# nmichlo/mtg-vision

Hardware: AMD Instinct MI355X
Metric: cards/sec end-to-end (detect+embed+top-1 over 100k bank), 640x640 (higher is better)
Workload: dtype f32 (products as 3 x f16 MFMA on hi/lo-split operands, f32 accumulate)

## Files before the change

mtg-vision_amd/csrc/dwconv7_ln_kernel.h:

```cpp
#pragma once
#include "common.h"
#include "dwconv7_ln_stream_kernel.h"
#include "sp8.h"

namespace mtgv {

typedef float f32x4 __attribute__((ext_vector_type(4)));

template <int TW, bool SP8, int PK, bool WL = false>
__global__ __launch_bounds__(256) void dwconv7_ln_kernel(const float* __restrict__ in, const float* __restrict__ w49,
                                                        const float* __restrict__ bias, const float* __restrict__ ln_w,
                                                        const float* __restrict__ ln_b, float* __restrict__ out, int H, int W,
                                                        int C, int nstrips, long total_strips, int S, float eps) {
  extern __shared__ __attribute__((aligned(16))) float sm[];
  const int c4n = C >> 2;
  float* part = sm;
  float* stat = sm + S * TW * c4n;
  const float* wl = w49;
  long blk;
  {
    const long nwg = gridDim.x, b = blockIdx.x;
    const long q = nwg >> 3, r = nwg & 7, x = b & 7;
    blk = (x < r ? x * (q + 1) : r * (q + 1) + (x - r) * q) + (b >> 3);
  }
  const int tid = threadIdx.x;
  if (WL) {
    float* wdst = stat + ((S * TW * 2 + 3) & ~3);
    for (int i = tid; i < 49 * c4n; i += 256) reinterpret_cast<f32x4*>(wdst)[i] = reinterpret_cast<const f32x4*>(w49)[i];
    wl = wdst;
    __syncthreads();
  }
  const int sl = tid / c4n, c4 = tid % c4n;
  const long strip = blk * S + sl;
  const bool live = sl < S && strip < total_strips;
  const int c = c4 * 4;
  int ws = 0, h = 0;
  long n = 0;
  if (live) {
    ws = (int)(strip % nstrips);
    const long t = strip / nstrips;
    h = (int)(t % H);
    n = t / H;
  }
  const int w0 = ws * TW;
  f32x4 acc[TW];
  if (live) {
    const f32x4 bv = *reinterpret_cast<const f32x4*>(bias + c);
#pragma unroll
    for (int j = 0; j < TW; ++j) acc[j] = bv;
#ifndef DW_DBG
#define DW_DBG 0
#endif
#pragma unroll 1
    for (int kh = 0; kh < 7; ++kh) {
      const int ih = h + kh - 3;
      if (ih < 0 || ih >= H) continue;
      if (DW_DBG == 1 && kh != 3) continue;
      const float* rowp = in + ((n * H + ih) * W) * C + c;
      f32x4 r[TW + 6];
#pragma unroll
      for (int j = 0; j < TW + 6; ++j) {
        const int iw = w0 + j - 3;
        f32x4 v = {0.f, 0.f, 0.f, 0.f};
        if (iw >= 0 && iw < W) v = *reinterpret_cast<const f32x4*>(rowp + (long)iw * C);
        r[j] = v;
      }
#pragma unroll
      for (int kw = 0; kw < 7; ++kw) {
        const f32x4 wv = *reinterpret_cast<const f32x4*>(wl + (kh * 7 + kw) * C + c);
#pragma unroll
        for (int j = 0; j < TW; ++j) {
          if (DW_DBG == 2) acc[j] += (kw == 0 ? r[j] + r[j + 6] : wv);
          else acc[j] += r[j + kw] * wv;
        }
      }
    }
#pragma unroll
    for (int j = 0; j < TW; ++j) part[(sl * c4n + c4) * TW + j] = (acc[j][0] + acc[j][1]) + (acc[j][2] + acc[j][3]);
  }
  __syncthreads();
  if (live && c4 < TW) {
    const float* pp = part + sl * c4n * TW + c4;
    float sum = 0.f;
    for (int i = 0; i < c4n; ++i) sum += pp[i * TW];
    stat[(sl * TW + c4) * 2] = sum / (float)C;
  }
  __syncthreads();
  if (live) {
#pragma unroll
    for (int j = 0; j < TW; ++j) {
      const f32x4 d = acc[j] - stat[(sl * TW + j) * 2];
      part[(sl * c4n + c4) * TW + j] = (d[0] * d[0] + d[1] * d[1]) + (d[2] * d[2] + d[3] * d[3]);
    }
  }
  __syncthreads();
  if (live && c4 < TW) {
    const float* pp = part + sl * c4n * TW + c4;
    float sq = 0.f;
    for (int i = 0; i < c4n; ++i) sq += pp[i * TW];
    stat[(sl * TW + c4) * 2 + 1] = 1.0f / sqrtf(sq / (float)C + eps);
  }
  __syncthreads();
  if (live) {
    const f32x4 wv = *reinterpret_cast<const f32x4*>(ln_w + c);
    const f32x4 bv = *reinterpret_cast<const f32x4*>(ln_b + c);
    float* op = out + ((n * H + h) * W + w0) * C + c;
#pragma unroll
    for (int j = 0; j < TW; ++j)
      if (w0 + j < W) {
        const float mean = stat[(sl * TW + j) * 2], rstd = stat[(sl * TW + j) * 2 + 1];
        const f32x4 o = (acc[j] - mean) * rstd * wv + bv;
        if (SP8)
          *reinterpret_cast<sp_h8*>(reinterpret_cast<char*>(op + (long)j * C - c) + (c4 >> 1) * 32 + (c4 & 1) * 16) =
              sp8_piece_from_quad(o, c4);
        else
          *reinterpret_cast<f32x4*>(op + (long)j * C) = o;
      }
  }
}


template <int TW, int TH, bool SP8, bool WL = false>
__global__ __launch_bounds__(256) void dwconv7_ln_rows_kernel(const float* __restrict__ in, const float* __restrict__ w49,
                                                             const float* __restrict__ bias, const float* __restrict__ ln_w,
                                                             const float* __restrict__ ln_b, float* __restrict__ out, int H, int W,
                                                             int C, int nstrips, int nhg, long total_strips, int S, float eps) {
  extern __shared__ __attribute__((aligned(16))) float sm[];
  constexpr int P = TH * TW;
  const int c4n = C >> 2;
  float* part = sm;
  float* stat = sm + S * P * c4n;
  const float* wl = w49;
  const int tid = threadIdx.x;
  if (WL) {
    float* wdst = stat + ((S * P * 2 + 3) & ~3);
    for (int i = tid; i < 49 * c4n; i += 256) reinterpret_cast<f32x4*>(wdst)[i] = reinterpret_cast<const f32x4*>(w49)[i];
    wl = wdst;
    __syncthreads();
  }
  const int sl = tid / c4n, c4 = tid % c4n;
  const int c = c4 * 4;
  long blk;
  {
    const long nwg = gridDim.x, b = blockIdx.x;
    const long q = nwg >> 3, r = nwg & 7, x = b & 7;
    blk = (x < r ? x * (q + 1) : r * (q + 1) + (x - r) * q) + (b >> 3);
  }
  const long strip = blk * S + sl;
  const bool live = sl < S && strip < total_strips;
  int ws = 0, h0 = 0;
  long n = 0;
  if (live) {
    ws = (int)(strip % nstrips);
    const long t = strip / nstrips;
    h0 = (int)(t % nhg) * TH;
    n = t / nhg;
  }
  const int w0 = ws * TW;
  f32x4 acc[TH][TW];
  if (live) {
    const f32x4 bv = *reinterpret_cast<const f32x4*>(bias + c);
#pragma unroll
    for (int t = 0; t < TH; ++t)
#pragma unroll
      for (int j = 0; j < TW; ++j) acc[t][j] = bv;
#pragma unroll 1
    for (int ir = 0; ir < TH + 6; ++ir) {
      const int ih = h0 + ir - 3;
      if (ih < 0 || ih >= H) continue;
      const float* rowp = in + ((n * H + ih) * W) * C + c;
      f32x4 r[TW + 6];
#pragma unroll
      for (int j = 0; j < TW + 6; ++j) {
        const int iw = w0 + j - 3;
        f32x4 v = {0.f, 0.f, 0.f, 0.f};
        if (iw >= 0 && iw < W) v = *reinterpret_cast<const f32x4*>(rowp + (long)iw * C);
        r[j] = v;
      }
#pragma unroll
      for (int t = 0; t < TH; ++t) {
        const int kh = ir - t;
        if (kh < 0 || kh > 6) continue;
#pragma unroll
        for (int kw = 0; kw < 7; ++kw) {
          const f32x4 wv = *reinterpret_cast<const f32x4*>(wl + (kh * 7 + kw) * C + c);
#pragma unroll
          for (int j = 0; j < TW; ++j) acc[t][j] += r[j + kw] * wv;
        }
      }
    }
#pragma unroll
    for (int t = 0; t < TH; ++t)
#pragma unroll
      for (int j = 0; j < TW; ++j)
        part[(sl * c4n + c4) * P + t * TW + j] = (acc[t][j][0] + acc[t][j][1]) + (acc[t][j][2] + acc[t][j][3]);
  }
  __syncthreads();
  if (live)
    for (int p = c4; p < P; p += c4n) {
      const float* pp = part + sl * c4n * P + p;
      float sum = 0.f;
      for (int i = 0; i < c4n; ++i) sum += pp[i * P];
      stat[(sl * P + p) * 2] = sum / (float)C;
    }
  __syncthreads();
  if (live) {
#pragma unroll
    for (int t = 0; t < TH; ++t)
#pragma unroll
      for (int j = 0; j < TW; ++j) {
        const f32x4 d = acc[t][j] - stat[(sl * P + t * TW + j) * 2];
        part[(sl * c4n + c4) * P + t * TW + j] = (d[0] * d[0] + d[1] * d[1]) + (d[2] * d[2] + d[3] * d[3]);
      }
  }
  __syncthreads();
  if (live)
    for (int p = c4; p < P; p += c4n) {
      const float* pp = part + sl * c4n * P + p;
      float sq = 0.f;
      for (int i = 0; i < c4n; ++i) sq += pp[i * P];
      stat[(sl * P + p) * 2 + 1] = 1.0f / sqrtf(sq / (float)C + eps);
    }
  __syncthreads();
  if (live) {
    const f32x4 wv = *reinterpret_cast<const f32x4*>(ln_w + c);
    const f32x4 bv = *reinterpret_cast<const f32x4*>(ln_b + c);
#pragma unroll
    for (int t = 0; t < TH; ++t) {
      if (h0 + t >= H) continue;
      float* op = out + ((n * H + h0 + t) * W + w0) * C + c;
#pragma unroll
      for (int j = 0; j < TW; ++j)
        if (w0 + j < W) {
          const float mean = stat[(sl * P + t * TW + j) * 2], rstd = stat[(sl * P + t * TW + j) * 2 + 1];
          const f32x4 o = (acc[t][j] - mean) * rstd * wv + bv;
          if (SP8)
            *reinterpret_cast<sp_h8*>(reinterpret_cast<char*>(op + (long)j * C - c) + (c4 >> 1) * 32 + (c4 & 1) * 16) =
                sp8_piece_from_quad(o, c4);
          else
            *reinterpret_cast<f32x4*>(op + (long)j * C) = o;
        }
    }
  }
}

template <int TW, int TH, bool SP8, bool WL = false>
static void dwconv7_ln_rows_launch(const float* in, const float* w49, const float* bias, const float* ln_w, const float* ln_b,
                                   float* out, int N, int H, int W, int C, float eps, hipStream_t s) {
  const int nstrips = ceil_div(W, TW), nhg = ceil_div(H, TH);
  const int c4n = C / 4;
  const int S = 256 / c4n;
  const long total_strips = (long)N * nhg * nstrips;
  const unsigned grid = (unsigned)((total_strips + S - 1) / S);
  const size_t lds = (size_t)(S * TH * TW * (c4n + 2) + 4 + (WL ? 49 * C : 0)) * sizeof(float);
  if (lds > 65536) {
    static bool attr[MTGV_MAX_DEVICES] = {};
    const int dev = current_device();
    if (!attr[dev]) {
      HIP_OK(hipFuncSetAttribute(reinterpret_cast<const void*>(&dwconv7_ln_rows_kernel<TW, TH, SP8, WL>), hipFuncAttributeMaxDynamicSharedMemorySize, 160 * 1024));
      attr[dev] = true;
    }
  }
  hipLaunchKernelGGL((dwconv7_ln_rows_kernel<TW, TH, SP8, WL>), dim3(grid), dim3(256), lds, s, in, w49, bias, ln_w, ln_b, out, H, W, C,
                     nstrips, nhg, total_strips, S, eps);
  HIP_OK(hipGetLastError());
}

template <int PK>
static void dwconv7_ln_launch_t(const float* in, const float* w49, const float* bias, const float* ln_w, const float* ln_b,
                                float* out, int N, int H, int W, int C, float eps, hipStream_t s, int out_fmt) {
  const char* const rows_env = getenv("MTGV_DW_ROWS");
  const bool rows_on = !(rows_env && atoi(rows_env) == 0);
  if constexpr (PK == 0)
  if (rows_on && N >= 128) {
#define DWSTREAM_GO(C_, G_)                                                                                                \
  (out_fmt == 1 ? dwconv7_ln_stream_launch<C_, G_, 4, 3, true>(in, w49, bias, ln_w, ln_b, out, N, H, 1, eps, s)            \
                : dwconv7_ln_stream_launch<C_, G_, 4, 3, false>(in, w49, bias, ln_w, ln_b, out, N, H, 1, eps, s))
    if (C == 96 && W == 32) { DWSTREAM_GO(96, 8); return; }
    if (C == 192 && W == 16) { DWSTREAM_GO(192, 4); return; }
#undef DWSTREAM_GO
  }
  if constexpr (PK == 0)
  if (rows_on && W >= 4) {
    const int c4n_ = C / 4, S_ = 256 / c4n_;
    const bool table = (size_t)(S_ * 12 * (c4n_ + 2) + 4 + 49 * C) * sizeof(float) <= 65536;
#define DWROWS_GO(TW_, WL_)                                                                                          \
  (out_fmt == 1 ? dwconv7_ln_rows_launch<TW_, 3, true, WL_>(in, w49, bias, ln_w, ln_b, out, N, H, W, C, eps, s)        \
                : dwconv7_ln_rows_launch<TW_, 3, false, WL_>(in, w49, bias, ln_w, ln_b, out, N, H, W, C, eps, s))
    if (table) DWROWS_GO(4, true);
    else if (W >= 8) DWROWS_GO(8, false);
    else DWROWS_GO(4, false);
#undef DWROWS_GO
    return;
  }
  const int tw = W >= 8 ? 8 : (W >= 4 ? 4 : 2);
  const int nstrips = ceil_div(W, tw);
  const int c4n = C / 4;
  const int S = 256 / c4n;
  const long total_strips = (long)N * H * nstrips;
  const unsigned grid = (unsigned)((total_strips + S - 1) / S);
  const size_t lds = (size_t)(S * tw * c4n + S * tw * 2) * sizeof(float);
#define DWLN_GO(TW_, SP_) \
  hipLaunchKernelGGL((dwconv7_ln_kernel<TW_, SP_, PK>), dim3(grid), dim3(256), lds, s, in, w49, bias, ln_w, ln_b, out, H, W, C, nstrips, total_strips, S, eps)
  if (out_fmt == 1) {
    if (tw == 8) DWLN_GO(8, true);
    else if (tw == 4) DWLN_GO(4, true);
    else DWLN_GO(2, true);
  } else {
    if (tw == 8) DWLN_GO(8, false);
    else if (tw == 4) DWLN_GO(4, false);
    else DWLN_GO(2, false);
  }
#undef DWLN_GO
  HIP_OK(hipGetLastError());
}

}
```

Baseline: 32540.

## Add whole-image LDS dwconv7+LayerNorm kernel for deep ConvNeXt stages

```diff
diff --git a/mtg-vision_amd/csrc/dwconv7_ln_image_kernel.h b/mtg-vision_amd/csrc/dwconv7_ln_image_kernel.h
--- /dev/null
+++ b/mtg-vision_amd/csrc/dwconv7_ln_image_kernel.h
@@ -0,0 +1,173 @@
+#pragma once
+#include <type_traits>
+
+#include "common.h"
+#include "sp8.h"
+
+namespace mtgv {
+
+template <int I, int N, typename F>
+__device__ __forceinline__ void dwi_static_for(F&& f) {
+  if constexpr (I < N) {
+    f(std::integral_constant<int, I>{});
+    dwi_static_for<I + 1, N>(f);
+  }
+}
+
+template <int C, int H, int W, int SPLIT, bool SP8>
+__global__ __launch_bounds__(C* SPLIT) void dwconv7_ln_image_kernel(const float* __restrict__ in, const float* __restrict__ w49,
+                                                                   const float* __restrict__ bias, const float* __restrict__ ln_w,
+                                                                   const float* __restrict__ ln_b, float* __restrict__ out, float eps) {
+  constexpr int NT = C * SPLIT, NW = NT / 64, TH = H / SPLIT, ROWF = W * C, PT = H * W, C4N = C / 4;
+  constexpr int DPW = ROWF * 4 / 1024 / NW;
+  constexpr int PITCH = C4N + 4;
+  constexpr int RB = 8;
+  constexpr int PPW = (PT + NW - 1) / NW;
+  constexpr int G = NT / C4N, PG = PT / G;
+  constexpr int LAST0 = (SPLIT - 1) * TH - 3 > 0 ? (SPLIT - 1) * TH - 3 : 0;
+  constexpr int PRE = LAST0 + 1;
+  static_assert(H % SPLIT == 0 && (SPLIT == 1 || (SPLIT == 2 && TH >= 3)), "bands must run the same number of row steps");
+  static_assert(NT % 256 == 0 && NT <= 1024 && C % 64 == 0, "every SIMD carries the same number of waves; a wave is in one band");
+  static_assert(ROWF * 4 % (1024 * NW) == 0 && H * DPW < 64, "whole DMA pieces per wave and row; counts fit s_waitcnt");
+  static_assert(PT * PITCH + 2 * PT <= H * ROWF && PPW <= 64 && PT % 4 == 0 && C4N % (4 * RB) == 0, "LayerNorm scratch reuses the image's LDS");
+  static_assert(NT % C4N == 0 && PT % G == 0 && C4N % 2 == 0, "whole pixel groups; SP8 lane pairs");
+  extern __shared__ __attribute__((aligned(1024))) char dwi_smem[];
+  float* const img = reinterpret_cast<float*>(dwi_smem);
+  float* const part = img;
+  float* const smean = img + PT * PITCH;
+  float* const srstd = smean + PT;
+  const int tid = threadIdx.x, lane = tid & 63;
+  const int wave = __builtin_amdgcn_readfirstlane(tid >> 6);
+  const int band = __builtin_amdgcn_readfirstlane(tid / C);
+  const int ch = tid - band * C;
+  const int h0 = band * TH;
+  const long n = blockIdx.x;
+  const char* const src = reinterpret_cast<const char*>(in + n * H * ROWF);
+
+  auto issue_rows = [&](int r0, int r1) {
+    for (int r = r0; r < r1; ++r)
+#pragma unroll
+      for (int k = 0; k < DPW; ++k) {
+        const int piece = k * NW + wave;
+        sp_dma16_saddr(src, (uint32_t)((r * ROWF + piece * 256 + lane * 4) * 4), reinterpret_cast<const char*>(img + r * ROWF + piece * 256));
+      }
+  };
+  issue_rows(0, PRE);
+  float wt[49];
+#pragma unroll
+  for (int t = 0; t < 49; ++t) wt[t] = w49[t * C + ch];
+  float bv = bias[ch];
+#pragma unroll
+  for (int t = 0; t < 49; ++t) asm volatile("" : "+v"(wt[t]));
+  asm volatile("" : "+v"(bv));
+  issue_rows(PRE, H);
+
+  float acc[TH][W];
+#pragma unroll
+  for (int t = 0; t < TH; ++t)
+#pragma unroll
+    for (int j = 0; j < W; ++j) acc[t][j] = bv;
+
+  auto conv_band = [&](auto BAND_T) {
+    constexpr int B = decltype(BAND_T)::value;
+    constexpr int H0 = B * TH, LO = H0 - 3 > 0 ? H0 - 3 : 0, HI = H0 + TH + 3 < H ? H0 + TH + 3 : H;
+    dwi_static_for<0, HI - LO>([&](auto K_T) {
+      constexpr int k = decltype(K_T)::value, ih = LO + k;
+      constexpr int need = LAST0 + k < H - 1 ? LAST0 + k : H - 1;
+      if constexpr (k == 0 || LAST0 + k <= H - 1) {
+        asm volatile("s_waitcnt vmcnt(%0)" ::"n"((H - 1 - need) * DPW) : "memory");
+        __syncthreads();
+      }
+      const float* const rowp = img + ih * ROWF + ch;
+      float r[W];
+#pragma unroll
+      for (int j = 0; j < W; ++j) r[j] = rowp[j * C];
+#pragma unroll
+      for (int t = 0; t < TH; ++t) {
+        const int kh = ih - (H0 + t) + 3;
+        if (kh < 0 || kh > 6) continue;
+#pragma unroll
+        for (int kw = 0; kw < 7; ++kw)
+#pragma unroll
+          for (int j = 0; j < W; ++j) {
+            const int jj = j + kw - 3;
+            if (jj < 0 || jj >= W) continue;
+            acc[t][j] = __builtin_fmaf(r[jj], wt[kh * 7 + kw], acc[t][j]);
+          }
+      }
+    });
+  };
+  if (SPLIT == 1 || band == 0) conv_band(std::integral_constant<int, 0>{});
+  else conv_band(std::integral_constant<int, SPLIT - 1>{});
+
+  __syncthreads();
+#pragma unroll
+  for (int t = 0; t < TH; ++t)
+#pragma unroll
+    for (int j = 0; j < W; ++j) img[((h0 + t) * W + j) * C + ch] = acc[t][j];
+  __syncthreads();
+  const int g = tid / C4N, q4 = tid - g * C4N;
+  sp_f4 v[PG];
+#pragma unroll
+  for (int i = 0; i < PG; ++i) v[i] = *reinterpret_cast<const sp_f4*>(img + (g * PG + i) * C + q4 * 4);
+  __syncthreads();
+#pragma unroll
+  for (int i = 0; i < PG; ++i) part[(g * PG + i) * PITCH + q4] = (v[i][0] + v[i][1]) + (v[i][2] + v[i][3]);
+  __syncthreads();
+  const int rp = wave * PPW + lane;
+  const bool reducer = lane < PPW && rp < PT;
+  auto quad_chain = [&]() {
+    const sp_f4* const pp = reinterpret_cast<const sp_f4*>(part + rp * PITCH);
+    constexpr int NB = C4N / 4 / RB;
+    float sum = 0.f;
+#pragma unroll 1
+    for (int b = 0; b < NB; ++b) {
+      sp_f4 cur[RB];
+#pragma unroll
+      for (int i = 0; i < RB; ++i) cur[i] = pp[b * RB + i];
+#pragma unroll
+      for (int i = 0; i < RB; ++i) sum += cur[i][0], sum += cur[i][1], sum += cur[i][2], sum += cur[i][3];
+    }
+    return sum;
+  };
+  if (reducer) smean[rp] = quad_chain() / (float)C;
+  __syncthreads();
+#pragma unroll
+  for (int i = 0; i < PG; ++i) {
+    const sp_f4 d = v[i] - smean[g * PG + i];
+    part[(g * PG + i) * PITCH + q4] = (d[0] * d[0] + d[1] * d[1]) + (d[2] * d[2] + d[3] * d[3]);
+  }
+  __syncthreads();
+  if (reducer) srstd[rp] = 1.0f / sqrtf(quad_chain() / (float)C + eps);
+  __syncthreads();
+  const sp_f4 lw = *reinterpret_cast<const sp_f4*>(ln_w + q4 * 4), lb = *reinterpret_cast<const sp_f4*>(ln_b + q4 * 4);
+#pragma unroll
+  for (int i = 0; i < PG; ++i) {
+    const int p = g * PG + i;
+    const float mean = smean[p], rstd = srstd[p];
+    const sp_f4 o = (v[i] - mean) * rstd * lw + lb;
+    float* const op = out + (n * PT + p) * C;
+    if (SP8)
+      *reinterpret_cast<sp_h8*>(reinterpret_cast<char*>(op) + (q4 >> 1) * 32 + (q4 & 1) * 16) = sp8_piece_from_quad(o, q4);
+    else
+      *reinterpret_cast<sp_f4*>(op + q4 * 4) = o;
+  }
+}
+
+template <int C, int H, int W, int SPLIT, bool SP8>
+static void dwconv7_ln_image_launch(const float* in, const float* w49, const float* bias, const float* ln_w, const float* ln_b, float* out,
+                                    int N, float eps, hipStream_t s) {
+  constexpr size_t lds = (size_t)H * W * C * sizeof(float);
+  static_assert(lds <= 160 * 1024, "the image must fit one CU's LDS");
+  auto kern = dwconv7_ln_image_kernel<C, H, W, SPLIT, SP8>;
+  static bool attr[MTGV_MAX_DEVICES] = {};
+  const int dev = current_device();
+  if (!attr[dev]) {
+    HIP_OK(hipFuncSetAttribute(reinterpret_cast<const void*>(kern), hipFuncAttributeMaxDynamicSharedMemorySize, 160 * 1024));
+    attr[dev] = true;
+  }
+  hipLaunchKernelGGL(kern, dim3((unsigned)N), dim3(C * SPLIT), lds, s, in, w49, bias, ln_w, ln_b, out, eps);
+  HIP_OK(hipGetLastError());
+}
+
+}
diff --git a/mtg-vision_amd/csrc/dwconv7_ln_kernel.h b/mtg-vision_amd/csrc/dwconv7_ln_kernel.h
--- a/mtg-vision_amd/csrc/dwconv7_ln_kernel.h
+++ b/mtg-vision_amd/csrc/dwconv7_ln_kernel.h
@@ -1,5 +1,6 @@
 #pragma once
 #include "common.h"
+#include "dwconv7_ln_image_kernel.h"
 #include "dwconv7_ln_stream_kernel.h"
 #include "sp8.h"
 
@@ -134,7 +135,7 @@
   const int tid = threadIdx.x;
   if (WL) {
     float* wdst = stat + ((S * P * 2 + 3) & ~3);
-    for (int i = tid; i < 49 * c4n; i += 256) reinterpret_cast<f32x4*>(wdst)[i] = reinterpret_cast<const f32x4*>(w49)[i];
+    for (int i = tid; i < 49 * c4n; i += blockDim.x) reinterpret_cast<f32x4*>(wdst)[i] = reinterpret_cast<const f32x4*>(w49)[i];
     wl = wdst;
     __syncthreads();
   }
@@ -261,7 +262,8 @@
       attr[dev] = true;
     }
   }
-  hipLaunchKernelGGL((dwconv7_ln_rows_kernel<TW, TH, SP8, WL>), dim3(grid), dim3(256), lds, s, in, w49, bias, ln_w, ln_b, out, H, W, C,
+  const unsigned threads = (unsigned)((S * c4n + 63) / 64 * 64);
+  hipLaunchKernelGGL((dwconv7_ln_rows_kernel<TW, TH, SP8, WL>), dim3(grid), dim3(threads), lds, s, in, w49, bias, ln_w, ln_b, out, H, W, C,
                      nstrips, nhg, total_strips, S, eps);
   HIP_OK(hipGetLastError());
 }
@@ -271,6 +273,17 @@
                                 float* out, int N, int H, int W, int C, float eps, hipStream_t s, int out_fmt) {
   const char* const rows_env = getenv("MTGV_DW_ROWS");
   const bool rows_on = !(rows_env && atoi(rows_env) == 0);
+  const char* const image_env = getenv("MTGV_DW_IMAGE");
+  const int image_mode = image_env ? atoi(image_env) : -1;
+  if constexpr (PK == 0)
+  if (rows_on && image_mode != 0 && (N >= 128 || image_mode == 1)) {
+#define DWIMAGE_GO(C_, H_, W_, SPLIT_)                                                                                    \
+  (out_fmt == 1 ? dwconv7_ln_image_launch<C_, H_, W_, SPLIT_, true>(in, w49, bias, ln_w, ln_b, out, N, eps, s)            \
+                : dwconv7_ln_image_launch<C_, H_, W_, SPLIT_, false>(in, w49, bias, ln_w, ln_b, out, N, eps, s))
+    if (C == 384 && H == 12 && W == 8) { DWIMAGE_GO(384, 12, 8, 2); return; }
+    if (C == 768 && H == 6 && W == 4) { DWIMAGE_GO(768, 6, 4, 1); return; }
+#undef DWIMAGE_GO
+  }
   if constexpr (PK == 0)
   if (rows_on && N >= 128) {
 #define DWSTREAM_GO(C_, G_)                                                                                                \
```

Measured after the change: 32920 (median of 6 runs). +1.2%, better.
